# mit-han-lab/distrifuser

Hardware: NVIDIA H100
Metric: SDXL 50-step latency (ms/image) (lower is better)
Workload: dtype f16

## Files before the change

distrifuser_b200/_lib.py:

```python
from __future__ import annotations

import ctypes as C
import os

HERE = os.path.dirname(os.path.abspath(__file__))
LIB_PATH = os.environ.get("DF_LIB_PATH") or os.path.join(HERE, "libdistrifuser_b200.so")

NBANKS = 3
MAX_WORLD = 8
IPC_HANDLE_BYTES = 64
TENSORMAP_BYTES = 128

EXPORTS = (
    "df_last_error", "df_version", "df_device_sm_count", "df_symm_alloc", "df_symm_open", "df_symm_close",
    "df_symm_free", "df_step_begin", "df_slot_publish", "df_slot_wait", "df_groupnorm_scratch_bytes",
    "df_groupnorm_fwd", "df_groupnorm_halo_fwd", "df_groupnorm_fwd_weighted", "df_groupnorm_halo_fwd_weighted", "df_halo_push",
    "df_halo_assemble", "df_attn_make_kvmaps", "df_attn_workspace_bytes", "df_attn_fwd", "df_attn_make_kvmaps_ragged",
    "df_attn_workspace_bytes_ragged", "df_attn_fwd_ragged",
    "df_output_gather", "df_output_gather_2d", "df_geglu", "df_add_layernorm", "df_bias_residual_add", "df_linear_supported", "df_linear_geglu_block", "df_linear_fwd",
)


class DfComm(C.Structure):
    _fields_ = [("base", C.c_void_p * MAX_WORLD), ("flags", C.c_void_p * MAX_WORLD), ("clock", C.c_void_p),
                ("tickets", C.c_void_p), ("bank_stride", C.c_uint64), ("spin_timeout_ns", C.c_uint64), ("world", C.c_int32),
                ("rank", C.c_int32)]


_lib = None


def lib():
    global _lib
    if _lib is None:
        if not os.path.exists(LIB_PATH):
            raise RuntimeError(
                f"{LIB_PATH} is missing: build it with `python -m distrifuser_b200.build` "
                "(distrifuser_b200 has no fallback path; the CUDA extension is the product)")
        L = C.CDLL(LIB_PATH)
        vp, u64, i32, u32, i64, f32 = C.c_void_p, C.c_uint64, C.c_int, C.c_uint32, C.c_int64, C.c_float
        L.df_last_error.restype = C.c_char_p
        L.df_version.restype = i32
        L.df_device_sm_count.argtypes = [C.POINTER(i32)]
        L.df_symm_alloc.argtypes = [C.c_size_t, C.POINTER(vp), vp]
        L.df_symm_open.argtypes = [vp, C.POINTER(vp)]
        L.df_symm_close.argtypes = [vp]
        L.df_symm_free.argtypes = [vp]
        L.df_step_begin.argtypes = [vp, i32, vp]
        L.df_slot_publish.argtypes = [DfComm, vp, u64, u64, u64, u64, u64, i32, u32, i32, vp]
        L.df_slot_wait.argtypes = [DfComm, i32, u32, vp]
        L.df_groupnorm_scratch_bytes.argtypes = [i32, i32, i32, i32, i32]
        L.df_groupnorm_scratch_bytes.restype = C.c_size_t
        L.df_groupnorm_fwd.argtypes = [DfComm, vp, vp, i64, vp, vp, vp, i32, i32, i32, i32, i32, f32, i32, i32, i32, i32, i32,
                                       u64, u64, u32, vp, vp]
        L.df_groupnorm_halo_fwd.argtypes = [DfComm, vp, vp, i64, vp, vp, vp, i32, i32, i32, i32, i32, f32, i32, i32, i32, i32, i32,
                                            u64, u64, u32, vp, i32, u64, u64, i32, i32, i32, i32, vp]
        i32p = C.POINTER(C.c_int32)
        L.df_groupnorm_fwd_weighted.argtypes = [DfComm, vp, vp, i64, vp, vp, vp, i32, i32, i32, i32, i32, f32, i32, i32, i32, i32,
                                                i32, u64, u64, u32, i32p, vp, vp]
        L.df_groupnorm_halo_fwd_weighted.argtypes = [DfComm, vp, vp, i64, vp, vp, vp, i32, i32, i32, i32, i32, f32, i32, i32, i32,
                                                     i32, i32, u64, u64, u32, i32p, vp, i32, u64, u64, i32, i32, i32, i32, vp]
        L.df_attn_make_kvmaps_ragged.argtypes = [DfComm, u64, u64, i32, i32p, i32, i32, vp, vp]
        L.df_attn_workspace_bytes_ragged.argtypes = [i32, i32, i32p, i32, i32, i32]
        L.df_attn_workspace_bytes_ragged.restype = C.c_size_t
        L.df_attn_fwd_ragged.argtypes = [DfComm, vp, vp, vp, vp, i32, i32, i32p, i32, i32, i64, i64, i64, i32, i32, i32p, i32,
                                         i32, f32, vp, C.c_size_t, vp]
        L.df_halo_push.argtypes = [DfComm, vp, i32, i32, i32, i32, i32, u64, u64, i32, i32, vp]
        L.df_halo_assemble.argtypes = [DfComm, vp, vp, i32, i32, i32, i32, i32, u64, u64, i32, i32, i32, vp]
        L.df_attn_make_kvmaps.argtypes = [DfComm, u64, u64, i32, i32, i32, i32, vp, vp]
        L.df_attn_workspace_bytes.argtypes = [i32, i32, i32, i32, i32, i32]
        L.df_attn_workspace_bytes.restype = C.c_size_t
        L.df_attn_fwd.argtypes = [DfComm, vp, vp, vp, vp, i32, i32, i32, i32, i32, i64, i64, i64, i32, i32,
                                  C.POINTER(C.c_int32), i32, i32, f32, vp, C.c_size_t, vp]
        L.df_geglu.argtypes = [vp, vp, i64, i32, i64, i64, vp]
        L.df_add_layernorm.argtypes = [vp, vp, vp, vp, vp, vp, i64, i32, f32, vp]
        L.df_bias_residual_add.argtypes = [vp, vp, vp, vp, i64, i32, vp]
        L.df_linear_supported.argtypes = [i64, i32, i32, i32]
        L.df_linear_geglu_block.argtypes = [i64, i32, i32]
        L.df_linear_fwd.argtypes = [DfComm, vp, vp, vp, vp, vp, i64, i32, i32, i64, i64, i64, i64, i32, i32, i32, i32, i32, u32, u64,
                                    u64, i32, vp]
        L.df_output_gather.argtypes = [DfComm, vp, vp, i32, i32, i32, i32, i32, i32, i32, i32, i32, u64, vp]
        L.df_output_gather_2d.argtypes = [DfComm, vp, vp, i32, i32, i32, i32, i32, i32, i32, i32, i32, i32, i32, u64, vp]
        for name in EXPORTS:
            getattr(L, name)
        _lib = L
    return _lib


KERNELS_PER_CALL = {"df_groupnorm_fwd": 1, "df_groupnorm_halo_fwd": 1, "df_attn_fwd": 1, "df_groupnorm_fwd_weighted": 1,
                    "df_groupnorm_halo_fwd_weighted": 1, "df_attn_fwd_ragged": 1, "df_halo_push": 1, "df_halo_assemble": 1,
                    "df_slot_publish": 1, "df_slot_wait": 1, "df_step_begin": 1, "df_output_gather": 2, "df_output_gather_2d": 2, "df_geglu": 1, "df_add_layernorm": 1, "df_bias_residual_add": 1,
                    "df_linear_fwd": 1}
LAUNCHES = {"total": 0}
PROFILE = None


def check(rc: int, what: str = ""):
    LAUNCHES["total"] += KERNELS_PER_CALL.get(what, 0)
    if rc != 0:
        raise RuntimeError(f"distrifuser_b200 {what} failed ({rc}): {lib().df_last_error().decode()}")


def int32_array(values) -> C.Array:
    values = list(values)
    assert len(values) <= MAX_WORLD
    return (C.c_int32 * MAX_WORLD)(*values)


def null_comm() -> DfComm:
    c = DfComm()
    c.world, c.rank, c.bank_stride = 1, 0, 0
    return c
```

distrifuser_b200/csrc/linear.cu:

```cuda
#include <math.h>
#include <string.h>

#include "tc_ptx.cuh"

using namespace df;
using namespace df::tc;

namespace {

constexpr int BM = 128;
constexpr int BK = 64;
constexpr int NTHREADS = 288;
constexpr int NCONSUMER_WARPS = 8;
constexpr uint32_t A_BYTES = BM * BK * 2;

template <int BN> struct Stages { static constexpr int value = BN == 256 ? 4 : 5; };

template <int BN>
struct __align__(1024) SmemT {
  __half a[Stages<BN>::value][BM * BK];
  __half b[Stages<BN>::value][BN * BK];
  uint64_t full[Stages<BN>::value], empty[Stages<BN>::value];
};

enum { EPI_PLAIN = 0, EPI_GEGLU = 1 };

struct LinearArgs {
  const __half* bias;
  const __half* residual;
  __half* out;
  int64_t M;
  int N, K;
  int64_t ldr, ldo;
  int tiles_m, tiles_n;
  int publish;
  int pub_col0, pub_cols;
  int idx;
  uint32_t peer_mask;
  uint64_t tensor_off, slot_bytes;
  df_comm_t comm;
};

__device__ __forceinline__ float gelu_erf(float x) {
  const float z = fabsf(x) * 0.70710678118654752f;
  const float t = __fdividef(1.f, fmaf(0.3275911f, z, 1.f));
  float p = fmaf(1.061405429f, t, -1.453152027f);
  p = fmaf(p, t, 1.421413741f);
  p = fmaf(p, t, -0.284496736f);
  p = fmaf(p, t, 0.254829592f);
  const float e = p * t * __expf(-z * z);
  const float phi = x >= 0.f ? 1.f - 0.5f * e : 0.5f * e;
  return x * phi;
}

__device__ __forceinline__ float2 ld_h2f(const __half* p) { return __half22float2(*reinterpret_cast<const __half2*>(p)); }

template <int BN>
__device__ __forceinline__ void wgmma_tile(float* acc, uint64_t a_desc, uint64_t b_desc, uint32_t accumulate) {
  if constexpr (BN == 256) wgmma_ss_n256(acc, a_desc, b_desc, accumulate);
  else wgmma_ss_n160(acc, a_desc, b_desc, accumulate);
}

template <int EPI, int BN>
__global__ void __launch_bounds__(NTHREADS, 1)
linear_kernel(const __grid_constant__ CUtensorMap tm_a, const __grid_constant__ CUtensorMap tm_w, LinearArgs p) {
  static_assert(BN % 32 == 0 && BN <= 256 && (BN * BK * 2) % 1024 == 0, "tile shape");
  constexpr int STAGES = Stages<BN>::value;
  constexpr uint32_t B_BYTES = BN * BK * 2;
  using Smem = SmemT<BN>;
  extern __shared__ __align__(1024) uint8_t smem_raw[];
  Smem& sm = *reinterpret_cast<Smem*>(smem_raw);
  if ((smem_u32(smem_raw) & 1023u) != 0) __trap();
  const int warp = threadIdx.x >> 5, lane = threadIdx.x & 31;
  const int ntiles = p.tiles_m * p.tiles_n;
  const int kblocks = p.K / BK;

  if (threadIdx.x == 0) {
    for (int s = 0; s < STAGES; ++s) { mbar_init(&sm.full[s], 1); mbar_init(&sm.empty[s], NCONSUMER_WARPS); }
    asm volatile("fence.mbarrier_init.release.cluster;" ::: "memory");
  }
  __syncthreads();
  pdl_wait();

  if (warp == NCONSUMER_WARPS) {
    if (lane == 0) {
      prefetch_tmap(&tm_a);
      prefetch_tmap(&tm_w);
      uint32_t stage = 0, phase = 0;
      for (int tile = blockIdx.x; tile < ntiles; tile += gridDim.x) {
        const int tm = tile % p.tiles_m, tn = tile / p.tiles_m;
        for (int kb = 0; kb < kblocks; ++kb) {
          mbar_wait(&sm.empty[stage], phase ^ 1u);
          mbar_expect_tx(&sm.full[stage], A_BYTES + B_BYTES);
          tma_load_2d(sm.a[stage], &tm_a, &sm.full[stage], kb * BK, tm * BM);
          tma_load_2d(sm.b[stage], &tm_w, &sm.full[stage], kb * BK, tn * BN);
          if (++stage == STAGES) { stage = 0; phase ^= 1u; }
        }
      }
    }
  } else {
    const int wg = warp >> 2;
    const int c4 = lane & 3;
    const int rloc = wg * 64 + (warp & 3) * 16 + (lane >> 2);
    uint32_t pub_epoch = 0;
    if (p.publish) pub_epoch = p.comm.clock[0];
    uint32_t stage = 0, phase = 0;
    float acc[BN / 2];
    for (int tile = blockIdx.x; tile < ntiles; tile += gridDim.x) {
      const int tm = tile % p.tiles_m, tn = tile / p.tiles_m;
      fence_regs<BN / 2>(acc);
      uint32_t prev = 0;
      for (int kb = 0; kb < kblocks; ++kb) {
        mbar_wait(&sm.full[stage], phase);
        const uint32_t a_addr = smem_u32(sm.a[stage]) + wg * 64 * 128, b_addr = smem_u32(sm.b[stage]);
        wgmma_fence();
#pragma unroll
        for (int kk = 0; kk < BK / 16; ++kk)
          wgmma_tile<BN>(acc, smem_desc(a_addr + kk * 32, 16, 1024), smem_desc(b_addr + kk * 32, 16, 1024), (kb | kk) > 0);
        wgmma_commit();
        wgmma_wait<1>();
        if (kb > 0 && lane == 0) mbar_arrive(&sm.empty[prev]);
        prev = stage;
        if (++stage == STAGES) { stage = 0; phase ^= 1u; }
      }
      wgmma_wait<0>();
      fence_regs<BN / 2>(acc);
      if (lane == 0) mbar_arrive(&sm.empty[prev]);
#pragma unroll
      for (int h = 0; h < 2; ++h) {
        const int64_t grow = (int64_t)tm * BM + rloc + 8 * h;
        if (grow >= p.M) continue;
        if (EPI == EPI_GEGLU) {
          __half* dst = p.out + grow * p.ldo + tn * (BN / 2);
#pragma unroll
          for (int i = 0; i < BN / 16; ++i) {
            const int c = 8 * i + 2 * c4;
            float2 bh = make_float2(0.f, 0.f), bg = make_float2(0.f, 0.f);
            if (p.bias) { bh = ld_h2f(p.bias + tn * BN + c); bg = ld_h2f(p.bias + tn * BN + BN / 2 + c); }
            const float* hv = acc + 4 * i + 2 * h;
            const float* gv = acc + 4 * (i + BN / 16) + 2 * h;
            const float2 hf = __half22float2(__floats2half2_rn(hv[0] + bh.x, hv[1] + bh.y));
            const float2 gf = __half22float2(__floats2half2_rn(gv[0] + bg.x, gv[1] + bg.y));
            *reinterpret_cast<__half2*>(dst + c) = __floats2half2_rn(hf.x * gelu_erf(gf.x), hf.y * gelu_erf(gf.y));
          }
        } else {
          const int col0 = tn * BN;
          __half* dst = p.out + grow * p.ldo + col0;
          const __half* res = p.residual ? p.residual + grow * p.ldr + col0 : nullptr;
#pragma unroll
          for (int i = 0; i < BN / 8; ++i) {
            const int c = 8 * i + 2 * c4;
            const int col = col0 + c;
            if (col >= p.N) continue;
            float2 f = make_float2(acc[4 * i + 2 * h], acc[4 * i + 2 * h + 1]);
            if (p.bias) { const float2 bb = ld_h2f(p.bias + col); f.x += bb.x; f.y += bb.y; }
            __half2 o = __floats2half2_rn(f.x, f.y);
            if (res) o = __hadd2(o, *reinterpret_cast<const __half2*>(res + c));
            *reinterpret_cast<__half2*>(dst + c) = o;
            if (p.publish && col >= p.pub_col0) {
              const uint64_t off = slot_offset(p.comm, pub_epoch, p.tensor_off, p.slot_bytes, p.comm.rank) +
                                   ((uint64_t)grow * p.pub_cols + (col - p.pub_col0)) * 2;
              for (int q = 0; q < p.comm.world; ++q)
                if (p.peer_mask >> q & 1) *reinterpret_cast<__half2*>((char*)p.comm.base[q] + off) = o;
            }
          }
        }
      }
    }
  }
  if (p.publish) signal_when_last(p.comm, &p.comm.tickets[p.idx], gridDim.x, p.idx, p.peer_mask, p.comm.clock[0]);
}

int make_map2d(CUtensorMap* m, const void* base, int64_t rows, int K, int64_t pitch, int box_rows) {
  EncodeTiledFn enc = tensor_map_encoder();
  DF_REQUIRE(enc != nullptr, "cuTensorMapEncodeTiled is not available from this driver");
  cuuint64_t dims[2] = {(cuuint64_t)K, (cuuint64_t)rows};
  cuuint64_t strides[1] = {(cuuint64_t)pitch * 2};
  cuuint32_t box[2] = {BK, (cuuint32_t)box_rows};
  cuuint32_t estr[2] = {1, 1};
  CUresult r = enc(m, CU_TENSOR_MAP_DATA_TYPE_FLOAT16, 2, const_cast<void*>(base), dims, strides, box, estr,
                   CU_TENSOR_MAP_INTERLEAVE_NONE, CU_TENSOR_MAP_SWIZZLE_128B, CU_TENSOR_MAP_L2_PROMOTION_L2_256B,
                   CU_TENSOR_MAP_FLOAT_OOB_FILL_NONE);
  DF_REQUIRE(r == CUDA_SUCCESS, "cuTensorMapEncodeTiled failed (%d): base=%p rows=%lld K=%d pitch=%lld", (int)r, base,
             (long long)rows, K, (long long)pitch);
  return 0;
}

template <int EPI, int BN>
int launch_linear(const CUtensorMap& ta, const CUtensorMap& tw, const LinearArgs& args, int ctas, cudaStream_t st) {
  static bool attr_set = false;
  if (!attr_set) {
    DF_CHECK_CUDA(cudaFuncSetAttribute(linear_kernel<EPI, BN>, cudaFuncAttributeMaxDynamicSharedMemorySize, (int)sizeof(SmemT<BN>)));
    attr_set = true;
  }
  DF_CHECK_CUDA(launch_pdl(PDL_GEMM, linear_kernel<EPI, BN>, dim3(ctas), dim3(NTHREADS), sizeof(SmemT<BN>), st, ta, tw, args));
  return 0;
}

double tile_cost(int64_t M, int N, int bn, int ctas_avail) {
  const long long tm = (M + BM - 1) / BM, tn = (N + bn - 1) / bn, tiles = tm * tn;
  const long long rounds = (tiles + ctas_avail - 1) / ctas_avail;
  return (double)rounds * (bn + 64);
}

}

namespace {
int pick_bn(int64_t M, int N, int epilogue, int cap) {
  const bool ok160 = epilogue == EPI_PLAIN || N % 160 == 0, ok256 = epilogue == EPI_PLAIN || N % 256 == 0;
  if (!ok256) return ok160 ? 160 : 0;
  if (ok160 && tile_cost(M, N, 160, cap) < 0.97 * tile_cost(M, N, 256, cap)) return 160;
  return 256;
}
}

extern "C" int df_linear_supported(int64_t M, int N, int K, int epilogue) {
  if (M < 1 || N < 8 || N % 8 != 0 || K < BK || K % BK != 0) return 0;
  if (epilogue == EPI_GEGLU && pick_bn(M, N, epilogue, sm_count()) == 0) return 0;
  return 1;
}

extern "C" int df_linear_geglu_block(int64_t M, int N, int K) {
  (void)K;
  const int bn = pick_bn(M, N, EPI_GEGLU, sm_count());
  return bn / 2;
}

extern "C" int df_linear_fwd(df_comm_t comm, const void* a, const void* w, const void* bias, const void* residual, void* out,
                             int64_t M, int N, int K, int64_t lda, int64_t ldw, int64_t ldr, int64_t ldo, int epilogue,
                             int geglu_block, int publish, int pub_col0, int idx, uint32_t peer_mask, uint64_t tensor_off,
                             uint64_t slot_bytes, int max_ctas, void* stream) {
  DF_REQUIRE(epilogue == EPI_PLAIN || epilogue == EPI_GEGLU, "df_linear_fwd: unknown epilogue %d", epilogue);
  DF_REQUIRE(df_linear_supported(M, N, K, epilogue), "df_linear_fwd: unsupported shape M=%lld N=%d K=%d (N %% 8, K %% 64%s)",
             (long long)M, N, K, epilogue == EPI_GEGLU ? ", GEGLU: N % 256" : "");
  DF_REQUIRE(((uintptr_t)a % 16) == 0 && ((uintptr_t)w % 16) == 0 && ((uintptr_t)out % 16) == 0 && ((uintptr_t)bias % 16) == 0 &&
                 ((uintptr_t)residual % 16) == 0 && lda % 8 == 0 && ldw % 8 == 0 && ldo % 8 == 0 && ldr % 8 == 0,
             "df_linear_fwd: operands must be 16-byte aligned with pitches multiple of 8");
  DF_REQUIRE(!(publish && epilogue != EPI_PLAIN), "df_linear_fwd: publication is a plain-epilogue feature");
  LinearArgs args;
  memset(&args, 0, sizeof(args));
  args.bias = (const __half*)bias; args.residual = (const __half*)residual; args.out = (__half*)out;
  args.M = M; args.N = N; args.K = K; args.ldr = ldr; args.ldo = ldo;
  const int sms = sm_count();
  const int cap = max_ctas > 0 ? max_ctas : sms;
  int bn = pick_bn(M, N, epilogue, epilogue == EPI_GEGLU ? sms : cap);
  if (epilogue == EPI_GEGLU && geglu_block > 0) {
    DF_REQUIRE(geglu_block == 80 || geglu_block == 128, "df_linear_fwd: geglu_block must be 80 or 128");
    bn = 2 * geglu_block;
    DF_REQUIRE(N % bn == 0, "df_linear_fwd: interleave block %d does not tile N=%d", geglu_block, N);
  }
  args.tiles_m = (int)((M + BM - 1) / BM);
  args.tiles_n = (N + bn - 1) / bn;
  args.publish = publish && peer_mask != 0;
  args.comm = comm;
  if (args.publish) {
    DF_REQUIRE(pub_col0 >= 0 && pub_col0 < N && pub_col0 % 8 == 0, "df_linear_fwd: bad pub_col0");
    args.pub_col0 = pub_col0; args.pub_cols = N - pub_col0; args.idx = idx; args.peer_mask = peer_mask;
    args.tensor_off = tensor_off; args.slot_bytes = slot_bytes;
    DF_REQUIRE((uint64_t)M * args.pub_cols * 2 <= slot_bytes, "df_linear_fwd: published columns larger than the slot");
  }
  int ctas = args.tiles_m * args.tiles_n;
  if (ctas > cap) ctas = cap;
  if (ctas < 1) ctas = 1;
  CUtensorMap ta, tw;
  if (int rc = make_map2d(&ta, a, M, K, lda, BM)) return rc;
  if (int rc = make_map2d(&tw, w, N, K, ldw, bn)) return rc;
  cudaStream_t st = (cudaStream_t)stream;
  if (epilogue == EPI_GEGLU) {
    if (bn == 160) return launch_linear<EPI_GEGLU, 160>(ta, tw, args, ctas, st);
    return launch_linear<EPI_GEGLU, 256>(ta, tw, args, ctas, st);
  }
  if (bn == 160) return launch_linear<EPI_PLAIN, 160>(ta, tw, args, ctas, st);
  return launch_linear<EPI_PLAIN, 256>(ta, tw, args, ctas, st);
}
```

distrifuser_b200/csrc/tc_ptx.cuh:

```cuda
#pragma once
#include <cuda.h>

#include "common.cuh"

namespace df {
namespace tc {

__device__ __forceinline__ uint32_t smem_u32(const void* p) { return (uint32_t)__cvta_generic_to_shared(p); }

__device__ __forceinline__ void mbar_init(uint64_t* bar, uint32_t count) {
  asm volatile("mbarrier.init.shared::cta.b64 [%0], %1;" ::"r"(smem_u32(bar)), "r"(count));
}
__device__ __forceinline__ void mbar_expect_tx(uint64_t* bar, uint32_t bytes) {
  asm volatile("mbarrier.arrive.expect_tx.shared::cta.b64 _, [%0], %1;" ::"r"(smem_u32(bar)), "r"(bytes) : "memory");
}
__device__ __forceinline__ void mbar_arrive(uint32_t bar_addr) {
  asm volatile("mbarrier.arrive.shared::cta.b64 _, [%0];" ::"r"(bar_addr) : "memory");
}
__device__ __forceinline__ void mbar_arrive(uint64_t* bar) { mbar_arrive(smem_u32(bar)); }
#ifndef DF_TRYWAIT_HINT_NS
#define DF_TRYWAIT_HINT_NS 200000u
#endif
__device__ __forceinline__ bool mbar_try(uint32_t bar_addr, uint32_t parity) {
  uint32_t ok;
  asm volatile(
      "{\n\t.reg .pred p;\n\t"
      "mbarrier.try_wait.parity.shared::cta.b64 p, [%1], %2, %3;\n\t"
      "selp.u32 %0, 1, 0, p;\n\t}"
      : "=r"(ok)
      : "r"(bar_addr), "r"(parity), "r"(DF_TRYWAIT_HINT_NS)
      : "memory");
  return ok != 0;
}
__device__ __forceinline__ bool mbar_try(uint64_t* bar, uint32_t parity) { return mbar_try(smem_u32(bar), parity); }
__device__ __forceinline__ void mbar_wait(uint32_t bar, uint32_t parity) {
  if (mbar_try(bar, parity)) return;
  uint32_t polls = 0;
  uint64_t t0 = 0;
  while (!mbar_try(bar, parity)) {
    if ((++polls & 0x3FFu) == 0) {
      const uint64_t now = globaltimer_ns();
      if (t0 == 0) t0 = now;
      else if (now - t0 > 10000000000ull) {
#ifdef DF_MBAR_DEBUG
        printf("distrifuser_b200: mbarrier timeout (block %d,%d,%d thread %d bar@%u parity %u)\n", blockIdx.x, blockIdx.y, blockIdx.z,
               threadIdx.x, bar, parity);
#endif
        __trap();
      }
    }
  }
}

__device__ __forceinline__ void mbar_wait(uint64_t* bar, uint32_t parity) { mbar_wait(smem_u32(bar), parity); }

__device__ __forceinline__ void tma_load_4d(void* dst, const void* tmap, uint64_t* bar, int c0, int c1, int c2, int c3) {
  asm volatile(
      "cp.async.bulk.tensor.4d.shared::cluster.global.mbarrier::complete_tx::bytes [%0], [%1, {%3, %4, %5, %6}], [%2];"
      ::"r"(smem_u32(dst)), "l"((uint64_t)tmap), "r"(smem_u32(bar)), "r"(c0), "r"(c1), "r"(c2), "r"(c3)
      : "memory");
}
__device__ __forceinline__ void tma_load_2d(void* dst, const void* tmap, uint64_t* bar, int c0, int c1) {
  asm volatile(
      "cp.async.bulk.tensor.2d.shared::cluster.global.mbarrier::complete_tx::bytes [%0], [%1, {%3, %4}], [%2];"
      ::"r"(smem_u32(dst)), "l"((uint64_t)tmap), "r"(smem_u32(bar)), "r"(c0), "r"(c1)
      : "memory");
}
__device__ __forceinline__ void prefetch_tmap(const void* tmap) {
  asm volatile("prefetch.tensormap [%0];" ::"l"((uint64_t)tmap) : "memory");
}

__device__ __forceinline__ uint64_t smem_desc(uint32_t addr, uint32_t lbo_bytes, uint32_t sbo_bytes) {
  return (uint64_t)((addr & 0x3FFFFu) >> 4) | ((uint64_t)((lbo_bytes >> 4) & 0x3FFFu) << 16) |
         ((uint64_t)((sbo_bytes >> 4) & 0x3FFFu) << 32) | (1ull << 62);
}
__device__ __forceinline__ void wgmma_fence() { asm volatile("wgmma.fence.sync.aligned;" ::: "memory"); }
__device__ __forceinline__ void wgmma_commit() { asm volatile("wgmma.commit_group.sync.aligned;" ::: "memory"); }
template <int N>
__device__ __forceinline__ void wgmma_wait() { asm volatile("wgmma.wait_group.sync.aligned %0;" ::"n"(N) : "memory"); }
template <int N>
__device__ __forceinline__ void setmaxnreg_dec() { asm volatile("setmaxnreg.dec.sync.aligned.u32 %0;" ::"n"(N)); }
template <int N>
__device__ __forceinline__ void setmaxnreg_inc() { asm volatile("setmaxnreg.inc.sync.aligned.u32 %0;" ::"n"(N)); }
template <int ID, int COUNT>
__device__ __forceinline__ void named_bar_sync() { asm volatile("bar.sync %0, %1;" ::"n"(ID), "n"(COUNT) : "memory"); }
template <int ID, int COUNT>
__device__ __forceinline__ void named_bar_arrive() { asm volatile("bar.arrive %0, %1;" ::"n"(ID), "n"(COUNT) : "memory"); }
template <int N>
__device__ __forceinline__ void fence_regs(float* d) {
#pragma unroll
  for (int i = 0; i < N; ++i) asm volatile("" : "+f"(d[i])::"memory");
}

__device__ __forceinline__ void wgmma_ss_n64(float* d, uint64_t a_desc, uint64_t b_desc, uint32_t accumulate) {
  asm volatile(
      "{\n\t.reg .pred p;\n\tsetp.ne.b32 p, %34, 0;\n\t"
      "wgmma.mma_async.sync.aligned.m64n64k16.f32.f16.f16 {%0, %1, %2, %3, %4, %5, %6, %7, %8, %9, %10, %11, %12, %13, %14, %15, %16, %17, %18, %19, %20, %21, %22, %23, %24, %25, %26, %27, %28, %29, %30, %31}, %32, %33, p, 1, 1, 0, 0;\n\t}"
      : "+f"(d[0]), "+f"(d[1]), "+f"(d[2]), "+f"(d[3]), "+f"(d[4]), "+f"(d[5]), "+f"(d[6]), "+f"(d[7]), "+f"(d[8]), "+f"(d[9]), "+f"(d[10]), "+f"(d[11]), "+f"(d[12]), "+f"(d[13]), "+f"(d[14]), "+f"(d[15]), "+f"(d[16]), "+f"(d[17]), "+f"(d[18]), "+f"(d[19]), "+f"(d[20]), "+f"(d[21]), "+f"(d[22]), "+f"(d[23]), "+f"(d[24]), "+f"(d[25]), "+f"(d[26]), "+f"(d[27]), "+f"(d[28]), "+f"(d[29]), "+f"(d[30]), "+f"(d[31])
      : "l"(a_desc), "l"(b_desc), "r"(accumulate));
}
__device__ __forceinline__ void wgmma_ss_n128(float* d, uint64_t a_desc, uint64_t b_desc, uint32_t accumulate) {
  asm volatile(
      "{\n\t.reg .pred p;\n\tsetp.ne.b32 p, %66, 0;\n\t"
      "wgmma.mma_async.sync.aligned.m64n128k16.f32.f16.f16 {%0, %1, %2, %3, %4, %5, %6, %7, %8, %9, %10, %11, %12, %13, %14, %15, %16, %17, %18, %19, %20, %21, %22, %23, %24, %25, %26, %27, %28, %29, %30, %31, %32, %33, %34, %35, %36, %37, %38, %39, %40, %41, %42, %43, %44, %45, %46, %47, %48, %49, %50, %51, %52, %53, %54, %55, %56, %57, %58, %59, %60, %61, %62, %63}, %64, %65, p, 1, 1, 0, 0;\n\t}"
      : "+f"(d[0]), "+f"(d[1]), "+f"(d[2]), "+f"(d[3]), "+f"(d[4]), "+f"(d[5]), "+f"(d[6]), "+f"(d[7]), "+f"(d[8]), "+f"(d[9]), "+f"(d[10]), "+f"(d[11]), "+f"(d[12]), "+f"(d[13]), "+f"(d[14]), "+f"(d[15]), "+f"(d[16]), "+f"(d[17]), "+f"(d[18]), "+f"(d[19]), "+f"(d[20]), "+f"(d[21]), "+f"(d[22]), "+f"(d[23]), "+f"(d[24]), "+f"(d[25]), "+f"(d[26]), "+f"(d[27]), "+f"(d[28]), "+f"(d[29]), "+f"(d[30]), "+f"(d[31]), "+f"(d[32]), "+f"(d[33]), "+f"(d[34]), "+f"(d[35]), "+f"(d[36]), "+f"(d[37]), "+f"(d[38]), "+f"(d[39]), "+f"(d[40]), "+f"(d[41]), "+f"(d[42]), "+f"(d[43]), "+f"(d[44]), "+f"(d[45]), "+f"(d[46]), "+f"(d[47]), "+f"(d[48]), "+f"(d[49]), "+f"(d[50]), "+f"(d[51]), "+f"(d[52]), "+f"(d[53]), "+f"(d[54]), "+f"(d[55]), "+f"(d[56]), "+f"(d[57]), "+f"(d[58]), "+f"(d[59]), "+f"(d[60]), "+f"(d[61]), "+f"(d[62]), "+f"(d[63])
      : "l"(a_desc), "l"(b_desc), "r"(accumulate));
}

__device__ __forceinline__ void wgmma_ss_n160(float* d, uint64_t a_desc, uint64_t b_desc, uint32_t accumulate) {
  asm volatile(
      "{\n\t.reg .pred p;\n\tsetp.ne.b32 p, %82, 0;\n\t"
      "wgmma.mma_async.sync.aligned.m64n160k16.f32.f16.f16 {%0, %1, %2, %3, %4, %5, %6, %7, %8, %9, %10, %11, %12, %13, %14, %15, %16, %17, %18, %19, %20, %21, %22, %23, %24, %25, %26, %27, %28, %29, %30, %31, %32, %33, %34, %35, %36, %37, %38, %39, %40, %41, %42, %43, %44, %45, %46, %47, %48, %49, %50, %51, %52, %53, %54, %55, %56, %57, %58, %59, %60, %61, %62, %63, %64, %65, %66, %67, %68, %69, %70, %71, %72, %73, %74, %75, %76, %77, %78, %79}, %80, %81, p, 1, 1, 0, 0;\n\t}"
      : "+f"(d[0]), "+f"(d[1]), "+f"(d[2]), "+f"(d[3]), "+f"(d[4]), "+f"(d[5]), "+f"(d[6]), "+f"(d[7]), "+f"(d[8]), "+f"(d[9]), "+f"(d[10]), "+f"(d[11]), "+f"(d[12]), "+f"(d[13]), "+f"(d[14]), "+f"(d[15]), "+f"(d[16]), "+f"(d[17]), "+f"(d[18]), "+f"(d[19]), "+f"(d[20]), "+f"(d[21]), "+f"(d[22]), "+f"(d[23]), "+f"(d[24]), "+f"(d[25]), "+f"(d[26]), "+f"(d[27]), "+f"(d[28]), "+f"(d[29]), "+f"(d[30]), "+f"(d[31]), "+f"(d[32]), "+f"(d[33]), "+f"(d[34]), "+f"(d[35]), "+f"(d[36]), "+f"(d[37]), "+f"(d[38]), "+f"(d[39]), "+f"(d[40]), "+f"(d[41]), "+f"(d[42]), "+f"(d[43]), "+f"(d[44]), "+f"(d[45]), "+f"(d[46]), "+f"(d[47]), "+f"(d[48]), "+f"(d[49]), "+f"(d[50]), "+f"(d[51]), "+f"(d[52]), "+f"(d[53]), "+f"(d[54]), "+f"(d[55]), "+f"(d[56]), "+f"(d[57]), "+f"(d[58]), "+f"(d[59]), "+f"(d[60]), "+f"(d[61]), "+f"(d[62]), "+f"(d[63]), "+f"(d[64]), "+f"(d[65]), "+f"(d[66]), "+f"(d[67]), "+f"(d[68]), "+f"(d[69]), "+f"(d[70]), "+f"(d[71]), "+f"(d[72]), "+f"(d[73]), "+f"(d[74]), "+f"(d[75]), "+f"(d[76]), "+f"(d[77]), "+f"(d[78]), "+f"(d[79])
      : "l"(a_desc), "l"(b_desc), "r"(accumulate));
}

__device__ __forceinline__ void wgmma_ss_n256(float* d, uint64_t a_desc, uint64_t b_desc, uint32_t accumulate) {
  asm volatile(
      "{\n\t.reg .pred p;\n\tsetp.ne.b32 p, %130, 0;\n\t"
      "wgmma.mma_async.sync.aligned.m64n256k16.f32.f16.f16 {%0, %1, %2, %3, %4, %5, %6, %7, %8, %9, %10, %11, %12, %13, %14, %15, %16, %17, %18, %19, %20, %21, %22, %23, %24, %25, %26, %27, %28, %29, %30, %31, %32, %33, %34, %35, %36, %37, %38, %39, %40, %41, %42, %43, %44, %45, %46, %47, %48, %49, %50, %51, %52, %53, %54, %55, %56, %57, %58, %59, %60, %61, %62, %63, %64, %65, %66, %67, %68, %69, %70, %71, %72, %73, %74, %75, %76, %77, %78, %79, %80, %81, %82, %83, %84, %85, %86, %87, %88, %89, %90, %91, %92, %93, %94, %95, %96, %97, %98, %99, %100, %101, %102, %103, %104, %105, %106, %107, %108, %109, %110, %111, %112, %113, %114, %115, %116, %117, %118, %119, %120, %121, %122, %123, %124, %125, %126, %127}, %128, %129, p, 1, 1, 0, 0;\n\t}"
// ... 36 lines not shown
```

distrifuser_b200/ops.py:

```python
import os as _os

import torch

from . import _lib


def geglu(y: torch.Tensor) -> torch.Tensor:
    assert y.is_cuda and y.dtype == torch.float16 and y.stride(-1) == 1
    cols = y.shape[-1] // 2
    y2 = y.reshape(-1, 2 * cols)
    out = torch.empty((*y.shape[:-1], cols), dtype=y.dtype, device=y.device)
    _lib.check(_lib.lib().df_geglu(y2.data_ptr(), out.data_ptr(), y2.shape[0], cols, y2.stride(0), cols,
                                   torch.cuda.current_stream().cuda_stream), "df_geglu")
    return out


def add_layernorm(x: torch.Tensor, r: torch.Tensor | None, norm: torch.nn.LayerNorm):
    assert x.is_cuda and x.dtype == torch.float16
    C = x.shape[-1]
    x = x.contiguous()
    y = torch.empty_like(x)
    if r is not None:
        r = r.contiguous()
        s = torch.empty_like(x)
    else:
        s = x
    _lib.check(_lib.lib().df_add_layernorm(x.data_ptr(), r.data_ptr() if r is not None else None,
                                           s.data_ptr() if r is not None else None, y.data_ptr(), norm.weight.data_ptr(),
                                           norm.bias.data_ptr(), x.numel() // C, C, float(norm.eps),
                                           torch.cuda.current_stream().cuda_stream), "df_add_layernorm")
    return s, y


def fused_conv_bias() -> bool:
    return _os.environ.get("DF_CONV_BIAS", "fused") != "torch"


def conv2d_bias_residual(x: torch.Tensor, conv: torch.nn.Conv2d, padding, residual: torch.Tensor | None = None,
                         bias: torch.Tensor | None = None, fold_bias: bool = False) -> torch.Tensor:
    import torch.nn.functional as F
    b = conv.bias if bias is None else bias
    ok = (x.is_cuda and x.dtype == torch.float16 and fused_conv_bias() and conv.out_channels % 8 == 0 and
          x.is_contiguous(memory_format=torch.channels_last))
    if not ok:
        out = F.conv2d(x, conv.weight, None if fold_bias else b, stride=conv.stride, padding=padding)
        return out if residual is None else residual + out
    out = F.conv2d(x, conv.weight, None, stride=conv.stride, padding=padding)
    if (b is None or fold_bias) and residual is None:
        return out
    if not out.is_contiguous(memory_format=torch.channels_last):
        out = out.contiguous(memory_format=torch.channels_last)
    if b is None or fold_bias:
        return residual + out
    if residual is not None:
        assert residual.shape == out.shape and residual.dtype == out.dtype
        if not residual.is_contiguous(memory_format=torch.channels_last):
            residual = residual.contiguous(memory_format=torch.channels_last)
    n, c, h, w = out.shape
    _lib.check(_lib.lib().df_bias_residual_add(out.data_ptr(), residual.data_ptr() if residual is not None else None,
                                               b.data_ptr(), out.data_ptr(), n * h * w, c,
                                               torch.cuda.current_stream().cuda_stream), "df_bias_residual_add")
    return out



_FUSED_LINEAR = set(_os.environ.get("DF_LINEAR", "geglu").replace("all", "geglu,qkv,out,ff2,proj").split(","))


def use_fused_linear(kind: str) -> bool:
    return kind in _FUSED_LINEAR


GEGLU_BLOCK = 128


def linear_supported(M: int, N: int, K: int, geglu: bool = False) -> bool:
    return bool(_lib.lib().df_linear_supported(M, N, K, 1 if geglu else 0))


def geglu_block(M: int, two_d: int, K: int) -> int:
    if not linear_supported(M, two_d, K, geglu=True):
        return 0
    return int(_lib.lib().df_linear_geglu_block(M, two_d, K))


def geglu_interleave(weight: torch.Tensor, bias: torch.Tensor | None, block: int = GEGLU_BLOCK):
    two_d, K = weight.shape
    D = two_d // 2
    assert D % block == 0
    w = torch.stack([weight[:D].reshape(D // block, block, K), weight[D:].reshape(D // block, block, K)], 1)
    w = w.reshape(two_d, K).contiguous()
    b = None
    if bias is not None:
        b = torch.stack([bias[:D].reshape(-1, block), bias[D:].reshape(-1, block)], 1).reshape(two_d).contiguous()
    return w, b


def linear(x: torch.Tensor, weight: torch.Tensor, bias: torch.Tensor | None = None, residual: torch.Tensor | None = None,
           out: torch.Tensor | None = None, publish=None) -> torch.Tensor:
# ... 33 lines not shown
```

include/distrifuser_b200.h:

```cpp
#ifndef DISTRIFUSER_B200_H
#define DISTRIFUSER_B200_H

#include <stddef.h>
#include <stdint.h>

#ifdef __cplusplus
extern "C" {
#endif

#define DF_NBANKS 3
#define DF_MAX_WORLD 8
#define DF_IPC_HANDLE_BYTES 64
#define DF_TENSORMAP_BYTES 128

const char* df_last_error(void);
int df_version(void);
int df_device_sm_count(int* out);

int df_symm_alloc(size_t bytes, void** dptr, void* ipc_handle_out_host );
int df_symm_open(const void* ipc_handle_host, void** peer_dptr);
int df_symm_close(void* peer_dptr);
int df_symm_free(void* dptr);

typedef struct {
// ... 30 lines not shown
int df_groupnorm_fwd_weighted(df_comm_t comm, const void* x, const void* addend, int64_t addend_pitch, void* y, const void* gamma,
                              const void* beta, int b, int h, int w, int C, int groups, float eps, int mode, int bessel,
                              int neg_var_fallback, int fuse_silu, int idx, uint64_t tensor_off, uint64_t slot_bytes,
                              uint32_t group_mask, const int32_t* src_weight_host , void* scratch, void* stream);
int df_groupnorm_halo_fwd_weighted(df_comm_t comm, const void* x, const void* addend, int64_t addend_pitch, void* y_padded,
                                   const void* gamma, const void* beta, int b, int h, int w, int C, int groups, float eps, int mode,
                                   int bessel, int neg_var_fallback, int fuse_silu, int idx, uint64_t tensor_off,
                                   uint64_t slot_bytes, uint32_t group_mask, const int32_t* src_weight_host ,
                                   void* scratch, int halo_idx, uint64_t halo_off, uint64_t halo_slot_bytes, int up_rank,
                                   int down_rank, int push, int wait_flags, void* stream);

int df_halo_push(df_comm_t comm, const void* x, int b, int h, int w, int C, int idx, uint64_t tensor_off,
                 uint64_t slot_bytes, int up_rank, int down_rank, void* stream);
int df_halo_assemble(df_comm_t comm, const void* x, void* xp, int b, int h, int w, int C, int idx,
                     uint64_t tensor_off, uint64_t slot_bytes, int up_rank, int down_rank, int wait_flags,
                     void* stream);

int df_attn_make_kvmaps(df_comm_t comm, uint64_t tensor_off, uint64_t slot_bytes, int b, int lseg, int heads,
                        int d, void* maps_out , void* stream);
size_t df_attn_workspace_bytes(int b, int lq, int lseg, int nseg, int heads, int d);
int df_attn_fwd(df_comm_t comm, const void* q, const void* kv_own, void* out, const void* kvmaps,
                int b, int lq, int lseg, int heads, int d, int64_t q_pitch, int64_t kv_pitch, int64_t o_pitch,
                int nseg, int own_seg, const int32_t* seg_rank_host, int idx, int wait_flags, float scale,
                void* workspace, size_t workspace_bytes, void* stream);
int df_attn_make_kvmaps_ragged(df_comm_t comm, uint64_t tensor_off, uint64_t slot_bytes, int b, const int32_t* seg_len_host,
                               int heads, int d, void* maps_out , void* stream);
size_t df_attn_workspace_bytes_ragged(int b, int lq, const int32_t* seg_len_host, int nseg, int heads, int d);
int df_attn_fwd_ragged(df_comm_t comm, const void* q, const void* kv_own, void* out, const void* kvmaps,
                       int b, int lq, const int32_t* seg_len_host, int heads, int d, int64_t q_pitch, int64_t kv_pitch,
                       int64_t o_pitch, int nseg, int own_seg, const int32_t* seg_rank_host, int idx, int wait_flags, float scale,
                       void* workspace, size_t workspace_bytes, void* stream);

int df_output_gather(df_comm_t comm, const void* strip, void* out, int B, int C, int H, int W, int bs, int hs,
                     int batch0, int row0, int idx, uint64_t tensor_off, void* stream);

int df_output_gather_2d(df_comm_t comm, const void* strip, void* out, int B, int C, int H, int W, int bs, int hs, int ws,
                        int batch0, int row0, int col0, int idx, uint64_t tensor_off, void* stream);

int df_geglu(const void* in, void* out, int64_t rows, int cols, int64_t in_pitch, int64_t out_pitch, void* stream);

int df_bias_residual_add(const void* a, const void* residual , const void* bias, void* out, int64_t rows, int C,
                         void* stream);

int df_add_layernorm(const void* x, const void* r, void* s_out, void* y, const void* gamma, const void* beta,
                     int64_t rows, int C, float eps, void* stream);

int df_linear_supported(int64_t M, int N, int K, int epilogue);
int df_linear_geglu_block(int64_t M, int N, int K);
int df_linear_fwd(df_comm_t comm, const void* a, const void* w, const void* bias, const void* residual, void* out,
                  int64_t M, int N, int K, int64_t lda, int64_t ldw, int64_t ldr, int64_t ldo, int epilogue,
                  int geglu_block, int publish, int pub_col0, int idx, uint32_t peer_mask, uint64_t tensor_off,
                  uint64_t slot_bytes, int max_ctas, void* stream);

#ifdef __cplusplus
}
#endif
#endif
```

Before: 1566.

## Add implicit-GEMM 3x3 conv kernel with fused bias and residual epilogue

```diff
diff --git a/distrifuser_b200/_lib.py b/distrifuser_b200/_lib.py
--- a/distrifuser_b200/_lib.py
+++ b/distrifuser_b200/_lib.py
@@ -18,6 +18,7 @@
     "df_halo_assemble", "df_attn_make_kvmaps", "df_attn_workspace_bytes", "df_attn_fwd", "df_attn_make_kvmaps_ragged",
     "df_attn_workspace_bytes_ragged", "df_attn_fwd_ragged",
     "df_output_gather", "df_output_gather_2d", "df_geglu", "df_add_layernorm", "df_bias_residual_add", "df_linear_supported", "df_linear_geglu_block", "df_linear_fwd",
+    "df_conv_supported", "df_conv3x3_fwd",
 )
 
 
@@ -79,6 +80,8 @@
         L.df_linear_geglu_block.argtypes = [i64, i32, i32]
         L.df_linear_fwd.argtypes = [DfComm, vp, vp, vp, vp, vp, i64, i32, i32, i64, i64, i64, i64, i32, i32, i32, i32, i32, u32, u64,
                                     u64, i32, vp]
+        L.df_conv_supported.argtypes = [i32, i32, i32, i32, i32, i32, i32]
+        L.df_conv3x3_fwd.argtypes = [vp, vp, vp, vp, vp, i32, i32, i32, i32, i32, i32, i32, i32, vp]
         L.df_output_gather.argtypes = [DfComm, vp, vp, i32, i32, i32, i32, i32, i32, i32, i32, i32, u64, vp]
         L.df_output_gather_2d.argtypes = [DfComm, vp, vp, i32, i32, i32, i32, i32, i32, i32, i32, i32, i32, i32, u64, vp]
         for name in EXPORTS:
@@ -90,7 +93,7 @@
 KERNELS_PER_CALL = {"df_groupnorm_fwd": 1, "df_groupnorm_halo_fwd": 1, "df_attn_fwd": 1, "df_groupnorm_fwd_weighted": 1,
                     "df_groupnorm_halo_fwd_weighted": 1, "df_attn_fwd_ragged": 1, "df_halo_push": 1, "df_halo_assemble": 1,
                     "df_slot_publish": 1, "df_slot_wait": 1, "df_step_begin": 1, "df_output_gather": 2, "df_output_gather_2d": 2, "df_geglu": 1, "df_add_layernorm": 1, "df_bias_residual_add": 1,
-                    "df_linear_fwd": 1}
+                    "df_linear_fwd": 1, "df_conv3x3_fwd": 1}
 LAUNCHES = {"total": 0}
 PROFILE = None
 
diff --git a/distrifuser_b200/csrc/linear.cu b/distrifuser_b200/csrc/linear.cu
--- a/distrifuser_b200/csrc/linear.cu
+++ b/distrifuser_b200/csrc/linear.cu
@@ -22,6 +22,16 @@
   __half b[Stages<BN>::value][BN * BK];
   uint64_t full[Stages<BN>::value], empty[Stages<BN>::value];
 };
+
+struct __align__(1024) SmemConv {
+  __half a[5][BM * BK];
+  __half b[5][160 * BK];
+  __half out[BM * 160];
+  uint64_t full[5], empty[5];
+  uint64_t res_full, out_free;
+};
+template <int BN, bool CONV> struct SmemOf { using type = SmemT<BN>; };
+template <> struct SmemOf<160, true> { using type = SmemConv; };
 
 enum { EPI_PLAIN = 0, EPI_GEGLU = 1 };
 
@@ -39,6 +49,8 @@
   uint32_t peer_mask;
   uint64_t tensor_off, slot_bytes;
   df_comm_t comm;
+  int cblocks;
+  int Ho, Wo, bh, bw_log2, ph, pw, tiles_x, tiles_y;
 };
 
 __device__ __forceinline__ float gelu_erf(float x) {
@@ -61,13 +73,21 @@
   else wgmma_ss_n160(acc, a_desc, b_desc, accumulate);
 }
 
-template <int EPI, int BN>
+struct ConvTile { int n, y0, x0; };
+__device__ __forceinline__ ConvTile conv_tile(const LinearArgs& p, int tm) {
+  const int tx = tm % p.tiles_x, t2 = tm / p.tiles_x;
+  return {t2 / p.tiles_y, (t2 % p.tiles_y) * p.bh, tx << p.bw_log2};
+}
+
+template <int EPI, int BN, bool CONV>
 __global__ void __launch_bounds__(NTHREADS, 1)
-linear_kernel(const __grid_constant__ CUtensorMap tm_a, const __grid_constant__ CUtensorMap tm_w, LinearArgs p) {
+linear_kernel(const __grid_constant__ CUtensorMap tm_a, const __grid_constant__ CUtensorMap tm_w,
+              const __grid_constant__ CUtensorMap tm_out, const __grid_constant__ CUtensorMap tm_res, LinearArgs p) {
   static_assert(BN % 32 == 0 && BN <= 256 && (BN * BK * 2) % 1024 == 0, "tile shape");
+  static_assert(!CONV || (EPI == EPI_PLAIN && BN == 160), "the convolution uses the plain epilogue on 160-wide tiles");
   constexpr int STAGES = Stages<BN>::value;
   constexpr uint32_t B_BYTES = BN * BK * 2;
-  using Smem = SmemT<BN>;
+  using Smem = typename SmemOf<BN, CONV>::type;
   extern __shared__ __align__(1024) uint8_t smem_raw[];
   Smem& sm = *reinterpret_cast<Smem*>(smem_raw);
   if ((smem_u32(smem_raw) & 1023u) != 0) __trap();
@@ -77,6 +97,7 @@
 
   if (threadIdx.x == 0) {
     for (int s = 0; s < STAGES; ++s) { mbar_init(&sm.full[s], 1); mbar_init(&sm.empty[s], NCONSUMER_WARPS); }
+    if constexpr (CONV) { mbar_init(&sm.res_full, 1); mbar_init(&sm.out_free, 1); }
     asm volatile("fence.mbarrier_init.release.cluster;" ::: "memory");
   }
   __syncthreads();
@@ -86,15 +107,30 @@
     if (lane == 0) {
       prefetch_tmap(&tm_a);
       prefetch_tmap(&tm_w);
-      uint32_t stage = 0, phase = 0;
-      for (int tile = blockIdx.x; tile < ntiles; tile += gridDim.x) {
+      uint32_t stage = 0, phase = 0, it = 0;
+      for (int tile = blockIdx.x; tile < ntiles; tile += gridDim.x, ++it) {
         const int tm = tile % p.tiles_m, tn = tile / p.tiles_m;
+        ConvTile ct{0, 0, 0};
+        if constexpr (CONV) ct = conv_tile(p, tm);
+        int cb = 0, r = 0, s = 0;
         for (int kb = 0; kb < kblocks; ++kb) {
           mbar_wait(&sm.empty[stage], phase ^ 1u);
           mbar_expect_tx(&sm.full[stage], A_BYTES + B_BYTES);
-          tma_load_2d(sm.a[stage], &tm_a, &sm.full[stage], kb * BK, tm * BM);
+          if constexpr (CONV) {
+            tma_load_4d(sm.a[stage], &tm_a, &sm.full[stage], cb * BK, ct.x0 + s - p.pw, ct.y0 + r - p.ph, ct.n);
+            if (++cb == p.cblocks) { cb = 0; if (++s == 3) { s = 0; ++r; } }
+          } else {
+            tma_load_2d(sm.a[stage], &tm_a, &sm.full[stage], kb * BK, tm * BM);
+          }
           tma_load_2d(sm.b[stage], &tm_w, &sm.full[stage], kb * BK, tn * BN);
           if (++stage == STAGES) { stage = 0; phase ^= 1u; }
+          if constexpr (CONV) {
+            if (kb == STAGES && p.residual) {
+              mbar_wait(&sm.out_free, (it & 1u) ^ 1u);
+              mbar_expect_tx(&sm.res_full, BM * BN * 2);
+              tma_load_4d(sm.out, &tm_res, &sm.res_full, tn * BN, ct.x0, ct.y0, ct.n);
+            }
+          }
         }
       }
     }
@@ -104,9 +140,9 @@
     const int rloc = wg * 64 + (warp & 3) * 16 + (lane >> 2);
     uint32_t pub_epoch = 0;
     if (p.publish) pub_epoch = p.comm.clock[0];
-    uint32_t stage = 0, phase = 0;
+    uint32_t stage = 0, phase = 0, it = 0;
     float acc[BN / 2];
-    for (int tile = blockIdx.x; tile < ntiles; tile += gridDim.x) {
+    for (int tile = blockIdx.x; tile < ntiles; tile += gridDim.x, ++it) {
       const int tm = tile % p.tiles_m, tn = tile / p.tiles_m;
       fence_regs<BN / 2>(acc);
       uint32_t prev = 0;
@@ -126,6 +162,38 @@
       wgmma_wait<0>();
       fence_regs<BN / 2>(acc);
       if (lane == 0) mbar_arrive(&sm.empty[prev]);
+      if constexpr (CONV) {
+        const int col0 = tn * BN;
+        __half2 bv[BN / 8];
+#pragma unroll
+        for (int i = 0; i < BN / 8; ++i)
+          bv[i] = p.bias && col0 + 8 * i + 2 * c4 < p.N ? __ldg(reinterpret_cast<const __half2*>(p.bias + col0 + 8 * i + 2 * c4))
+                                                         : __floats2half2_rn(0.f, 0.f);
+        named_bar_sync<1, NCONSUMER_WARPS * 32>();
+        if (p.residual) mbar_wait(&sm.res_full, it & 1u);
+#pragma unroll
+        for (int h = 0; h < 2; ++h) {
+          __half* o = sm.out + (rloc + 8 * h) * BN;
+#pragma unroll
+          for (int i = 0; i < BN / 8; ++i) {
+            const int c = 8 * i + 2 * c4;
+            float2 f = __half22float2(__floats2half2_rn(acc[4 * i + 2 * h], acc[4 * i + 2 * h + 1]));
+            const float2 bb = __half22float2(bv[i]);
+            f.x += bb.x; f.y += bb.y;
+            if (p.residual) { const float2 rr = __half22float2(*reinterpret_cast<const __half2*>(o + c)); f.x += rr.x; f.y += rr.y; }
+            *reinterpret_cast<__half2*>(o + c) = __floats2half2_rn(f.x, f.y);
+          }
+        }
+        fence_proxy_async_smem();
+        named_bar_sync<1, NCONSUMER_WARPS * 32>();
+        if (threadIdx.x == 0) {
+          const ConvTile ct = conv_tile(p, tm);
+          tma_store_4d(&tm_out, sm.out, col0, ct.x0, ct.y0, ct.n);
+          bulk_commit();
+          bulk_wait_read<0>();
+          mbar_arrive(&sm.out_free);
+        }
+      } else {
 #pragma unroll
       for (int h = 0; h < 2; ++h) {
         const int64_t grow = (int64_t)tm * BM + rloc + 8 * h;
@@ -166,8 +234,10 @@
           }
         }
       }
+      }
     }
   }
+  if constexpr (CONV) if (threadIdx.x == 0) bulk_wait<0>();
   if (p.publish) signal_when_last(p.comm, &p.comm.tickets[p.idx], gridDim.x, p.idx, p.peer_mask, p.comm.clock[0]);
 }
 
@@ -186,14 +256,31 @@
   return 0;
 }
 
-template <int EPI, int BN>
-int launch_linear(const CUtensorMap& ta, const CUtensorMap& tw, const LinearArgs& args, int ctas, cudaStream_t st) {
+int make_map_nhwc(CUtensorMap* m, const void* base, int N, int H, int W, int C, int box_c, int bw, int bh, bool swizzle) {
+  EncodeTiledFn enc = tensor_map_encoder();
+  DF_REQUIRE(enc != nullptr, "cuTensorMapEncodeTiled is not available from this driver");
+  cuuint64_t dims[4] = {(cuuint64_t)C, (cuuint64_t)W, (cuuint64_t)H, (cuuint64_t)N};
+  cuuint64_t strides[3] = {(cuuint64_t)C * 2, (cuuint64_t)W * C * 2, (cuuint64_t)H * W * C * 2};
+  cuuint32_t box[4] = {(cuuint32_t)box_c, (cuuint32_t)bw, (cuuint32_t)bh, 1};
+  cuuint32_t estr[4] = {1, 1, 1, 1};
+  CUresult r = enc(m, CU_TENSOR_MAP_DATA_TYPE_FLOAT16, 4, const_cast<void*>(base), dims, strides, box, estr,
+                   CU_TENSOR_MAP_INTERLEAVE_NONE, swizzle ? CU_TENSOR_MAP_SWIZZLE_128B : CU_TENSOR_MAP_SWIZZLE_NONE,
+                   CU_TENSOR_MAP_L2_PROMOTION_L2_256B,
+                   CU_TENSOR_MAP_FLOAT_OOB_FILL_NONE);
+  DF_REQUIRE(r == CUDA_SUCCESS, "cuTensorMapEncodeTiled failed (%d): base=%p N=%d H=%d W=%d C=%d", (int)r, base, N, H, W, C);
+  return 0;
+}
+
+template <int EPI, int BN, bool CONV = false>
+int launch_linear(const CUtensorMap& ta, const CUtensorMap& tw, const CUtensorMap& to, const CUtensorMap& tr,
+                  const LinearArgs& args, int ctas, cudaStream_t st) {
+  using Smem = typename SmemOf<BN, CONV>::type;
   static bool attr_set = false;
   if (!attr_set) {
-    DF_CHECK_CUDA(cudaFuncSetAttribute(linear_kernel<EPI, BN>, cudaFuncAttributeMaxDynamicSharedMemorySize, (int)sizeof(SmemT<BN>)));
+    DF_CHECK_CUDA(cudaFuncSetAttribute(linear_kernel<EPI, BN, CONV>, cudaFuncAttributeMaxDynamicSharedMemorySize, (int)sizeof(Smem)));
     attr_set = true;
   }
-  DF_CHECK_CUDA(launch_pdl(PDL_GEMM, linear_kernel<EPI, BN>, dim3(ctas), dim3(NTHREADS), sizeof(SmemT<BN>), st, ta, tw, args));
+  DF_CHECK_CUDA(launch_pdl(PDL_GEMM, linear_kernel<EPI, BN, CONV>, dim3(ctas), dim3(NTHREADS), sizeof(Smem), st, ta, tw, to, tr, args));
   return 0;
 }
 
@@ -267,9 +354,61 @@
   if (int rc = make_map2d(&tw, w, N, K, ldw, bn)) return rc;
   cudaStream_t st = (cudaStream_t)stream;
   if (epilogue == EPI_GEGLU) {
-    if (bn == 160) return launch_linear<EPI_GEGLU, 160>(ta, tw, args, ctas, st);
-    return launch_linear<EPI_GEGLU, 256>(ta, tw, args, ctas, st);
-  }
-  if (bn == 160) return launch_linear<EPI_PLAIN, 160>(ta, tw, args, ctas, st);
-  return launch_linear<EPI_PLAIN, 256>(ta, tw, args, ctas, st);
-}
+    if (bn == 160) return launch_linear<EPI_GEGLU, 160>(ta, tw, ta, ta, args, ctas, st);
+    return launch_linear<EPI_GEGLU, 256>(ta, tw, ta, ta, args, ctas, st);
+  }
+  if (bn == 160) return launch_linear<EPI_PLAIN, 160>(ta, tw, ta, ta, args, ctas, st);
+  return launch_linear<EPI_PLAIN, 256>(ta, tw, ta, ta, args, ctas, st);
+}
+
+extern "C" int df_conv_supported(int N, int H, int W, int Cin, int Cout, int ph, int pw) {
+  if (N < 1 || Cin < BK || Cin % BK != 0 || Cout < 8 || Cout % 8 != 0) return 0;
+  if (ph < 0 || ph > 1 || pw < 0 || pw > 1) return 0;
+  if (H + 2 * ph - 2 < 1 || W + 2 * pw - 2 < 1) return 0;
+  return 1;
+}
+
+extern "C" int df_conv3x3_fwd(const void* x, const void* w, const void* bias, const void* residual, void* out, int N, int H,
+                              int W, int Cin, int Cout, int ph, int pw, int max_ctas, void* stream) {
+  DF_REQUIRE(df_conv_supported(N, H, W, Cin, Cout, ph, pw),
+             "df_conv3x3_fwd: unsupported shape N=%d H=%d W=%d Cin=%d Cout=%d ph=%d pw=%d (Cin %% 64, Cout %% 8)", N, H, W, Cin,
+             Cout, ph, pw);
+  DF_REQUIRE(((uintptr_t)x % 16) == 0 && ((uintptr_t)w % 16) == 0 && ((uintptr_t)out % 16) == 0 && ((uintptr_t)bias % 16) == 0 &&
+                 ((uintptr_t)residual % 16) == 0,
+             "df_conv3x3_fwd: operands must be 16-byte aligned");
+  LinearArgs args;
+  memset(&args, 0, sizeof(args));
+  args.bias = (const __half*)bias; args.residual = (const __half*)residual; args.out = (__half*)out;
+  args.Ho = H + 2 * ph - 2; args.Wo = W + 2 * pw - 2;
+  args.ph = ph; args.pw = pw;
+  int bw = BM;
+  if (args.Wo < BM && BM % args.Wo == 0) bw = args.Wo;
+  const int bh = BM / bw;
+  int lg = 0;
+  while ((1 << lg) < bw) ++lg;
+  args.bw_log2 = lg; args.bh = bh;
+  args.tiles_x = (args.Wo + bw - 1) / bw;
+  args.tiles_y = (args.Ho + bh - 1) / bh;
+  args.cblocks = Cin / BK;
+  args.K = 9 * Cin; args.N = Cout;
+  args.M = (int64_t)N * args.Ho * args.Wo;
+  args.ldr = Cout; args.ldo = Cout;
+  const long long tiles_m = (long long)N * args.tiles_y * args.tiles_x;
+  DF_REQUIRE(tiles_m < (1ll << 30), "df_conv3x3_fwd: image too large");
+  args.tiles_m = (int)tiles_m;
+  const int cap = max_ctas > 0 ? max_ctas : sm_count();
+  constexpr int bn = 160;
+  args.tiles_n = (Cout + bn - 1) / bn;
+  args.comm.world = 1;
+  int ctas = args.tiles_m * args.tiles_n;
+  if (ctas > cap) ctas = cap;
+  if (ctas < 1) ctas = 1;
+  CUtensorMap ta, tw, to, tr;
+  if (int rc = make_map_nhwc(&ta, x, N, H, W, Cin, BK, bw, bh, true)) return rc;
+  if (int rc = make_map2d(&tw, w, Cout, 9 * Cin, 9 * (int64_t)Cin, bn)) return rc;
+  if (int rc = make_map_nhwc(&to, out, N, args.Ho, args.Wo, Cout, bn, bw, bh, false)) return rc;
+  tr = to;
+  if (residual)
+    if (int rc = make_map_nhwc(&tr, residual, N, args.Ho, args.Wo, Cout, bn, bw, bh, false)) return rc;
+  return launch_linear<EPI_PLAIN, bn, true>(ta, tw, to, tr, args, ctas, (cudaStream_t)stream);
+}
diff --git a/distrifuser_b200/csrc/tc_ptx.cuh b/distrifuser_b200/csrc/tc_ptx.cuh
--- a/distrifuser_b200/csrc/tc_ptx.cuh
+++ b/distrifuser_b200/csrc/tc_ptx.cuh
@@ -66,6 +66,17 @@
       ::"r"(smem_u32(dst)), "l"((uint64_t)tmap), "r"(smem_u32(bar)), "r"(c0), "r"(c1)
       : "memory");
 }
+__device__ __forceinline__ void tma_store_4d(const void* tmap, const void* src, int c0, int c1, int c2, int c3) {
+  asm volatile("cp.async.bulk.tensor.4d.global.shared::cta.bulk_group [%0, {%2, %3, %4, %5}], [%1];"
+               ::"l"((uint64_t)tmap), "r"(smem_u32(src)), "r"(c0), "r"(c1), "r"(c2), "r"(c3)
+               : "memory");
+}
+__device__ __forceinline__ void bulk_commit() { asm volatile("cp.async.bulk.commit_group;" ::: "memory"); }
+template <int N>
+__device__ __forceinline__ void bulk_wait_read() { asm volatile("cp.async.bulk.wait_group.read %0;" ::"n"(N) : "memory"); }
+template <int N>
+__device__ __forceinline__ void bulk_wait() { asm volatile("cp.async.bulk.wait_group %0;" ::"n"(N) : "memory"); }
+__device__ __forceinline__ void fence_proxy_async_smem() { asm volatile("fence.proxy.async.shared::cta;" ::: "memory"); }
 __device__ __forceinline__ void prefetch_tmap(const void* tmap) {
   asm volatile("prefetch.tensormap [%0];" ::"l"((uint64_t)tmap) : "memory");
 }
diff --git a/distrifuser_b200/ops.py b/distrifuser_b200/ops.py
--- a/distrifuser_b200/ops.py
+++ b/distrifuser_b200/ops.py
@@ -36,6 +36,57 @@
     return _os.environ.get("DF_CONV_BIAS", "fused") != "torch"
 
 
+def _conv_weight_rsc(conv: torch.nn.Conv2d) -> torch.Tensor:
+    w = conv.weight
+    if w.is_contiguous(memory_format=torch.channels_last):
+        return w.detach().permute(0, 2, 3, 1)
+    key = (w._version, w.data_ptr())
+    cache = getattr(conv, "_df_weight_rsc", None)
+    if cache is None or cache[0] != key:
+        if torch.cuda.is_current_stream_capturing():
+            raise RuntimeError("conv weight changed since the last eager call; run one eager call before capture")
+        with torch.no_grad():
+            cache = (key, w.detach().permute(0, 2, 3, 1).contiguous())
+        conv._df_weight_rsc = cache
+    return cache[1]
+
+
+CONV3X3_MAX_OUT = 2 * 128 * 128 * 320
+
+
+def conv3x3_supported(x: torch.Tensor, conv: torch.nn.Conv2d, padding) -> bool:
+    pad = tuple(padding) if isinstance(padding, (tuple, list)) else (padding, padding)
+    if not (x.is_cuda and x.dtype == torch.float16 and x.dim() == 4 and x.is_contiguous(memory_format=torch.channels_last)):
+        return False
+    if (tuple(conv.kernel_size) != (3, 3) or tuple(conv.stride) != (1, 1) or tuple(conv.dilation) != (1, 1) or conv.groups != 1
+            or conv.weight.dtype != torch.float16 or not all(isinstance(p, int) for p in pad) or pad[1] != 1 or pad[0] not in (0, 1)):
+        return False
+    n, c, h, w = x.shape
+    if n * (h + 2 * pad[0] - 2) * (w + 2 * pad[1] - 2) * conv.out_channels > CONV3X3_MAX_OUT:
+        return False
+    return bool(_lib.lib().df_conv_supported(n, h, w, c, conv.out_channels, pad[0], pad[1]))
+
+
+def conv3x3(x: torch.Tensor, conv: torch.nn.Conv2d, padding, bias: torch.Tensor | None = None,
+            residual: torch.Tensor | None = None) -> torch.Tensor:
+    pad = tuple(padding) if isinstance(padding, (tuple, list)) else (padding, padding)
+    n, c, h, w = x.shape
+    ho, wo = h + 2 * pad[0] - 2, w + 2 * pad[1] - 2
+    cout = conv.out_channels
+    out = torch.empty((n, cout, ho, wo), dtype=x.dtype, device=x.device, memory_format=torch.channels_last)
+    if residual is not None:
+        assert residual.shape == out.shape and residual.dtype == out.dtype
+        if not residual.is_contiguous(memory_format=torch.channels_last):
+            residual = residual.contiguous(memory_format=torch.channels_last)
+    if bias is not None:
+        assert bias.dtype == torch.float16 and bias.is_contiguous()
+    wk = _conv_weight_rsc(conv)
+    _lib.check(_lib.lib().df_conv3x3_fwd(x.data_ptr(), wk.data_ptr(), bias.data_ptr() if bias is not None else None,
+                                         residual.data_ptr() if residual is not None else None, out.data_ptr(), n, h, w, c, cout,
+                                         pad[0], pad[1], 0, torch.cuda.current_stream().cuda_stream), "df_conv3x3_fwd")
+    return out
+
+
 def conv2d_bias_residual(x: torch.Tensor, conv: torch.nn.Conv2d, padding, residual: torch.Tensor | None = None,
                          bias: torch.Tensor | None = None, fold_bias: bool = False) -> torch.Tensor:
     import torch.nn.functional as F
@@ -45,6 +96,8 @@
     if not ok:
         out = F.conv2d(x, conv.weight, None if fold_bias else b, stride=conv.stride, padding=padding)
         return out if residual is None else residual + out
+    if conv3x3_supported(x, conv, padding):
+        return conv3x3(x, conv, padding, None if fold_bias else b, residual)
     out = F.conv2d(x, conv.weight, None, stride=conv.stride, padding=padding)
     if (b is None or fold_bias) and residual is None:
         return out
diff --git a/include/distrifuser_b200.h b/include/distrifuser_b200.h
--- a/include/distrifuser_b200.h
+++ b/include/distrifuser_b200.h
@@ -106,6 +106,10 @@
                   int geglu_block, int publish, int pub_col0, int idx, uint32_t peer_mask, uint64_t tensor_off,
                   uint64_t slot_bytes, int max_ctas, void* stream);
 
+int df_conv_supported(int N, int H, int W, int Cin, int Cout, int ph, int pw);
+int df_conv3x3_fwd(const void* x, const void* w, const void* bias, const void* residual, void* out, int N, int H, int W,
+                   int Cin, int Cout, int ph, int pw, int max_ctas, void* stream);
+
 #ifdef __cplusplus
 }
 #endif
```

Measured after the change: 1542, median of 6. -1.5%, faster.
